# paolomandica/HALO

Measured on AMD Instinct MI355X. Metric: acquisition-scored images/sec (1024x2048, C=256, 19 cls), higher is better.
Workload: dtype f64

## Files before the change

halo_amd/csrc/halo_score.hip:

```cpp
#include "halo_common.hpp"
#include "halo_devmath.hpp"
#include "halo_select_plan.hpp"
#include "halo_softmax.hpp"
#include <stdlib.h>
#include <type_traits>

namespace halo {

constexpr int TPB = 256;
#ifndef HALO_FTPB
#define HALO_FTPB 128
#endif
#ifndef HALO_FEAT_WAVES
#define HALO_FEAT_WAVES 4
#endif
#ifndef HALO_FEAT_UNROLL
#define HALO_FEAT_UNROLL 8
#endif
constexpr int FTPB = HALO_FTPB;

__device__ __forceinline__ double nan_min(double a, double b) { return (a != a) ? a : ((b != b) ? b : (b < a ? b : a)); }
__device__ __forceinline__ double nan_max(double a, double b) { return (a != a) ? a : ((b != b) ? b : (b > a ? b : a)); }

template <int NT = TPB>
// ... 546 lines not shown
        unc[(size_t)b * hw + i] = a;
        mn = mx = (double)a;
    }
    if (!partials) return;
    __shared__ double seed[2];
    if (threadIdx.x == 0) { seed[0] = mn; seed[1] = mx; }
    __syncthreads();
    if (!live) { mn = seed[0]; mx = seed[1]; }
    block_minmax<TPB>(mn, mx, partials + ((size_t)b * gridDim.x + blockIdx.x) * 2);
}

__device__ __forceinline__ float lane_prev(float v)
{
    return __int_as_float(__builtin_amdgcn_update_dpp(0, __float_as_int(v), 0x138 , 0xf, 0xf, false));
}
__device__ __forceinline__ float lane_next(float v)
{
    return __int_as_float(__builtin_amdgcn_update_dpp(0, __float_as_int(v), 0x130 , 0xf, 0xf, false));
}

__device__ __forceinline__ float box3_over_count(float a, int H, int W, int y, int xx, int pk)
{
    if (pk <= 0) return a;
    const int rr = pk / 2;
    const int y0 = y - rr < 0 ? 0 : y - rr, y1 = y + rr >= H ? H - 1 : y + rr;
    const int x0 = xx - rr < 0 ? 0 : xx - rr, x1 = xx + rr >= W ? W - 1 : xx + rr;
    return a / (float)((y1 - y0 + 1) * (x1 - x0 + 1));
}

__device__ __forceinline__ void box3_row4(const float *__restrict__ ep, int H, int W, int y, int x, bool live, int pk, float (&o)[4])
{
    const int lane = threadIdx.x & 63;
    float r[3][6];
#pragma unroll
    for (int dy = 0; dy < 3; ++dy) {
        const int yy = y + dy - 1;
        const bool in = live && yy >= 0 && yy < H;
        const float *row = ep + (size_t)(in ? yy : 0) * W;
        float4 q = make_float4(0.0f, 0.0f, 0.0f, 0.0f);
        if (in) q = *reinterpret_cast<const float4 *>(row + x);
        float left = lane_prev(q.w), right = lane_next(q.x);
        if (lane == 0) left = (in && x > 0) ? row[x - 1] : 0.0f;
        if (lane == 63) right = (in && x + 4 < W) ? row[x + 4] : 0.0f;
        r[dy][0] = (in && x > 0) ? left : 0.0f;
        r[dy][1] = q.x; r[dy][2] = q.y; r[dy][3] = q.z; r[dy][4] = q.w;
        r[dy][5] = (in && x + 4 < W) ? right : 0.0f;
    }
#pragma unroll
    for (int j = 0; j < 4; ++j) {
        float a = 0.0f;
#pragma unroll
        for (int dy = 0; dy < 3; ++dy)
#pragma unroll
            for (int dx = 0; dx < 3; ++dx) a = a + r[dy][j + dx];
        o[j] = box3_over_count(a, H, W, y, x + j, pk);
    }
}

__global__ void __launch_bounds__(TPB) k_box3_unc(const float *__restrict__ ent, int H, int W, int pk,
                                                  float *__restrict__ unc, double *__restrict__ partials)
{
    const int b = blockIdx.y;
    const long long hw = (long long)H * W;
    const long long i0 = ((long long)blockIdx.x * TPB + threadIdx.x) * 4;
    const bool live = i0 < hw;
    double mn = 0.0, mx = 0.0;
    const int y = live ? (int)(i0 / W) : 0, x = live ? (int)(i0 % W) : 0;
    float o[4];
    box3_row4(ent + (size_t)b * hw, H, W, y, x, live, pk, o);
    if (live) {
        if (unc) *reinterpret_cast<float4 *>(unc + (size_t)b * hw + i0) = make_float4(o[0], o[1], o[2], o[3]);
        mn = mx = (double)o[0];
#pragma unroll
        for (int j = 1; j < 4; ++j) { mn = nan_min(mn, (double)o[j]); mx = nan_max(mx, (double)o[j]); }
    }
    if (!partials) return;
    __shared__ double seed[2];
    if (threadIdx.x == 0) { seed[0] = mn; seed[1] = mx; }
    __syncthreads();
    if (!live) { mn = seed[0]; mx = seed[1]; }
    block_minmax<TPB>(mn, mx, partials + ((size_t)b * gridDim.x + blockIdx.x) * 2);
}

constexpr int BM_RPT = 4, BM_TW = 256, BM_TH = BM_RPT * (TPB / 64);

__device__ __forceinline__ float nan_minf(float a, float b) { return (a != a) ? a : ((b != b) ? b : (b < a ? b : a)); }
__device__ __forceinline__ float nan_maxf(float a, float b) { return (a != a) ? a : ((b != b) ? b : (b > a ? b : a)); }

__global__ void __launch_bounds__(TPB) k_box3_minmax(const float *__restrict__ ent, int H, int W, int pk, double *__restrict__ partials,
                                                     unsigned *__restrict__ hist_zero)
{
    const int b = blockIdx.z, lane = threadIdx.x & 63, wv = threadIdx.x >> 6;
    if (hist_zero) {
        const unsigned nb = gridDim.x * gridDim.y;
        for (unsigned l = blockIdx.y * gridDim.x + blockIdx.x; l < NB1 / TPB; l += nb) hist_zero[(size_t)b * NB1 + l * TPB + threadIdx.x] = 0u;
    }
    const int x = blockIdx.x * BM_TW + lane * 4, y0 = blockIdx.y * BM_TH + wv * BM_RPT;
    const float *ep = ent + (size_t)b * H * W;
    const bool xin = x < W;
    auto load_row = [&](int yy, float (&r)[6]) {
        const bool in = xin && yy >= 0 && yy < H;
        const float *row = ep + (size_t)(in ? yy : 0) * W;
        float4 q = make_float4(0.0f, 0.0f, 0.0f, 0.0f);
        if (in) q = *reinterpret_cast<const float4 *>(row + x);
        float left = lane_prev(q.w), right = lane_next(q.x);
        if (lane == 0) left = (in && x > 0) ? row[x - 1] : 0.0f;
        if (lane == 63) right = (in && x + 4 < W) ? row[x + 4] : 0.0f;
        r[0] = (in && x > 0) ? left : 0.0f;
        r[1] = q.x; r[2] = q.y; r[3] = q.z; r[4] = q.w;
        r[5] = (in && x + 4 < W) ? right : 0.0f;
    };
    float r0[6], r1[6], r2[6];
    load_row(y0 - 1, r0);
    load_row(y0, r1);
    float mn = 0.0f, mx = 0.0f;
    bool have = false;
#pragma unroll
    for (int k = 0; k < BM_RPT; ++k) {
        const int y = y0 + k;
        load_row(y + 1, r2);
        if (xin && y < H) {
#pragma unroll
            for (int j = 0; j < 4; ++j) {
                float a = 0.0f;
#pragma unroll
                for (int dx = 0; dx < 3; ++dx) a = a + r0[j + dx];
#pragma unroll
                for (int dx = 0; dx < 3; ++dx) a = a + r1[j + dx];
#pragma unroll
                for (int dx = 0; dx < 3; ++dx) a = a + r2[j + dx];
                const float o = box3_over_count(a, H, W, y, x + j, pk);
                if (!have) { mn = mx = o; have = true; }
                else { mn = nan_minf(mn, o); mx = nan_maxf(mx, o); }
            }
        }
#pragma unroll
        for (int q = 0; q < 6; ++q) { r0[q] = r1[q]; r1[q] = r2[q]; }
    }
    __shared__ float seedf[2];
    __shared__ float smn[TPB / 64], smx[TPB / 64];
    if (threadIdx.x == 0) { seedf[0] = mn; seedf[1] = mx; }
    __syncthreads();
    if (!have) { mn = seedf[0]; mx = seedf[1]; }
#pragma unroll
    for (int off = 32; off > 0; off >>= 1) {
        mn = nan_minf(mn, __shfl_xor(mn, off));
        mx = nan_maxf(mx, __shfl_xor(mx, off));
    }
    if (lane == 0) { smn[wv] = mn; smx[wv] = mx; }
    __syncthreads();
    if (threadIdx.x == 0) {
#pragma unroll
        for (int i = 1; i < TPB / 64; ++i) { mn = nan_minf(mn, smn[i]); mx = nan_maxf(mx, smx[i]); }
        double *out2 = partials + (((size_t)b * gridDim.y + blockIdx.y) * gridDim.x + blockIdx.x) * 2;
        out2[0] = (double)mn;
        out2[1] = (double)mx;
    }
}

__global__ void __launch_bounds__(TPB) k_minmax_f32(const float *__restrict__ x, long long hw,
                                                    double *__restrict__ partials)
{
    const int b = blockIdx.y;
    const long long i = (long long)blockIdx.x * TPB + threadIdx.x;
    const bool live = i < hw;
    double mn = 0.0, mx = 0.0;
    if (live) mn = mx = (double)x[(size_t)b * hw + i];
    __shared__ double seed[2];
    if (threadIdx.x == 0) { seed[0] = mn; seed[1] = mx; }
    __syncthreads();
    if (!live) { mn = seed[0]; mx = seed[1]; }
    block_minmax<TPB>(mn, mx, partials + ((size_t)b * gridDim.x + blockIdx.x) * 2);
}

__global__ void __launch_bounds__(TPB) k_fill_f32(float *__restrict__ x, long long n, float v)
{
    const long long i = (long long)blockIdx.x * TPB + threadIdx.x;
    if (i < n) x[i] = v;
}

template <typename TI>
__global__ void __launch_bounds__(TPB) k_combine(const TI *__restrict__ imp_raw, const float *__restrict__ unc_raw,
                                                 const double *__restrict__ stats, const unsigned char *__restrict__ active,
                                                 long long hw, int normalize, TI *__restrict__ score,
                                                 TI *__restrict__ imp_out, float *__restrict__ unc_out)
{
    const int b = blockIdx.y;
    const long long i = (long long)blockIdx.x * TPB + threadIdx.x;
    if (i >= hw) return;
    const size_t o = (size_t)b * hw + i;
    TI im = imp_raw[o];
    float un = unc_raw[o];
    if (normalize) {
        const float umn = (float)stats[b * 4 + 2], umx = (float)stats[b * 4 + 3];
        un = (un - umn) / (float)((double)umx - (double)umn);
        const TI imn = (TI)stats[b * 4 + 0], imx = (TI)stats[b * 4 + 1];
        if constexpr (sizeof(TI) == 8) im = (im - imn) / (imx - imn);
        else im = (im - imn) / (float)((double)imx - (double)imn);
    }
    TI s = im * (TI)un;
    if (active && active[o]) {
        if constexpr (sizeof(TI) == 8) s = __longlong_as_double(0xfff0000000000000ll);
        else s = __uint_as_float(0xff800000u);
    }
    score[o] = s;
    if (imp_out) imp_out[o] = im;
    if (unc_out) unc_out[o] = un;
}


constexpr int CB_ROWS = 16;

template <typename TI>
__global__ void __launch_bounds__(TPB) k_combine_box3(const TI *__restrict__ imp_raw, const float *__restrict__ ent,
                                                      const double *__restrict__ stats, const unsigned char *__restrict__ active,
                                                      int H, int W, int pk, int normalize, TI *__restrict__ score,
                                                      TI *__restrict__ imp_out, float *__restrict__ unc_out, SelHdr *__restrict__ rng,
                                                      unsigned *__restrict__ hist, int rows)
{
    __shared__ unsigned hl[NB1];
    const int b = blockIdx.z;
    const long long hw = (long long)H * W;
    const int x = (blockIdx.x * TPB + threadIdx.x) * 4;
    const bool live = x < W;
    float umn = 0.0f, uden = 1.0f;
    TI imn = (TI)0, iden = (TI)1;
    bool fin = false;
    if (normalize) {
        umn = (float)stats[b * 4 + 2];
        const float umx = (float)stats[b * 4 + 3];
        uden = (float)((double)umx - (double)umn);
        imn = (TI)stats[b * 4 + 0];
        const TI imx = (TI)stats[b * 4 + 1];
        if constexpr (sizeof(TI) == 8) iden = imx - imn;
        else iden = (float)((double)imx - (double)imn);
        fin = uden > 0.0f && uden < __builtin_inff() && iden > (TI)0 && iden < (TI)__builtin_inf();
        if (rng && blockIdx.x == 0 && blockIdx.y == 0 && threadIdx.x == 0) {
            SelHdr h;
            memset(&h, 0, sizeof(h));
            h.kmin_inv = ~order_key(0.0);
            h.kmax = order_key(1.0);
            h.nvalid = 1u;
            h.flags = fin ? (hist ? (unsigned)SEL_F_HIST : 0u) : (unsigned)SEL_F_BAD;
            rng[b] = h;
        }
    }
    const bool count = hist != nullptr && fin;
    if (count) {
        for (int j = threadIdx.x; j < NB1; j += TPB) hl[j] = 0u;
        __syncthreads();
    }
    ValRange vr;
    vr.lo = 0.0; vr.scale = (double)NB1; vr.ok = true;
    const int ybeg = blockIdx.y * rows, yend = ybeg + rows < H ? ybeg + rows : H;
    const float *ep = ent + (size_t)b * hw;
    const int lane = threadIdx.x & 63;
    struct RowRaw { float4 q; float el, er; bool in; };
    auto row_issue = [&](int yy) {
        RowRaw t;
        t.in = live && yy >= 0 && yy < H;
        const float *row = ep + (size_t)(t.in ? yy : 0) * W;
        t.q = make_float4(0.0f, 0.0f, 0.0f, 0.0f);
        t.el = 0.0f; t.er = 0.0f;
        if (t.in) t.q = *reinterpret_cast<const float4 *>(row + x);
        if (lane == 0 && t.in && x > 0) t.el = row[x - 1];
        if (lane == 63 && t.in && x + 4 < W) t.er = row[x + 4];
        return t;
    };
    auto row_finish = [&](const RowRaw &t, float (&r)[6]) {
        float left = lane_prev(t.q.w), right = lane_next(t.q.x);
        if (lane == 0) left = t.el;
        if (lane == 63) right = t.er;
        r[0] = (t.in && x > 0) ? left : 0.0f;
        r[1] = t.q.x; r[2] = t.q.y; r[3] = t.q.z; r[4] = t.q.w;
        r[5] = (t.in && x + 4 < W) ? right : 0.0f;
    };
    typedef double cb_d2 __attribute__((ext_vector_type(2)));
    typedef float cb_f4 __attribute__((ext_vector_type(4)));
    struct PixRaw { cb_d2 d0, d1; cb_f4 f; unsigned am; };
    auto pix_issue = [&](int yy) {
        PixRaw t;
        t.d0 = (cb_d2){0.0, 0.0}; t.d1 = t.d0; t.f = (cb_f4){0.f, 0.f, 0.f, 0.f}; t.am = 0u;
        if (!live || yy >= yend) return t;
        const size_t o = (size_t)b * hw + (size_t)yy * W + x;
        if constexpr (sizeof(TI) == 8) {
            t.d0 = *reinterpret_cast<const cb_d2 *>(imp_raw + o);
            t.d1 = *reinterpret_cast<const cb_d2 *>(imp_raw + o + 2);
        } else {
            t.f = *reinterpret_cast<const cb_f4 *>(imp_raw + o);
        }
        if (active) t.am = *reinterpret_cast<const unsigned *>(active + o);
        return t;
    };
    float r0[6], r1[6], r2[6];
    {
        const RowRaw a0 = row_issue(ybeg - 1), a1 = row_issue(ybeg);
        row_finish(a0, r0);
        row_finish(a1, r1);
    }
    RowRaw nrow = row_issue(ybeg + 1);
    PixRaw npix = pix_issue(ybeg);
    for (int y = ybeg; y < yend; ++y) {
        row_finish(nrow, r2);
        const PixRaw cpix = npix;
        nrow = row_issue(y + 2);
        npix = pix_issue(y + 1);
        float un[4];
#pragma unroll
        for (int j = 0; j < 4; ++j) {
            float a = 0.0f;
#pragma unroll
            for (int dx = 0; dx < 3; ++dx) a = a + r0[j + dx];
#pragma unroll
            for (int dx = 0; dx < 3; ++dx) a = a + r1[j + dx];
#pragma unroll
            for (int dx = 0; dx < 3; ++dx) a = a + r2[j + dx];
// ... 840 lines not shown
    const Taps<float> ty = make_taps<float>(y, sh, h), tx = make_taps<float>(x, sw, w);
    const float *lb = logit + (size_t)b * bstride;
    for (int c = 0; c < O; ++c) {
        const float *pl = lb + (size_t)c * h * w;
        dst[((size_t)b * O + c) * hw + i] = bilerp<float>(pl[(size_t)ty.i0 * w + tx.i0], pl[(size_t)ty.i0 * w + tx.i1],
                                                          pl[(size_t)ty.i1 * w + tx.i0], pl[(size_t)ty.i1 * w + tx.i1], tx.l0, tx.l1, ty.l0, ty.l1);
    }
}

static inline bool aligned16(const void *p) { return ((uintptr_t)p & 15) == 0; }

struct FusedLogit { const float *logit; long long bstride; int O; int unc_type; float *ent; };

template <typename T, int VEC>
static void launch_feat(const T *feat, long long bstride, int C, long long hw, int B, int mode, double ks, double rks,
                        T *out, double *partials, int nblk, hipStream_t st, const FusedLogit *fl)
{
    dim3 grid(nblk, B), block(FTPB);
    constexpr int UNROLL = HALO_FEAT_UNROLL;
    unsigned xcd_g = 256;
    while (xcd_g > 1 && 8 * xcd_g > (unsigned)nblk) xcd_g >>= 1;
    if (8 * xcd_g > (unsigned)nblk) xcd_g = 0;
#define HALO_FEAT(M, FO_)                                                                                               \
    hipLaunchKernelGGL((k_feat_reduce<T, VEC, M, UNROLL, FO_>), grid, block, 0, st, feat, bstride, C, hw, ks, rks, out, \
                       partials, fl ? fl->logit : nullptr, fl ? fl->bstride : 0ll, fl ? fl->unc_type : 0, fl ? fl->ent : nullptr, \
                       xcd_g)
    const int fo = fl ? fl->O : 0;
    if (mode == 0) {
        if (fo == 19) HALO_FEAT(0, 19); else if (fo == 16) HALO_FEAT(0, 16); else HALO_FEAT(0, 0);
    } else {
        if (fo == 19) HALO_FEAT(1, 19); else if (fo == 16) HALO_FEAT(1, 16); else HALO_FEAT(1, 0);
    }
#undef HALO_FEAT
}

}

using namespace halo;

static_assert(RI_TW == LR_TW && RI_TH == LR_TH, "k_region_impurity3 writes one min/max partial per tile of the same shape");
static size_t partial_slots(int64_t H, int64_t W)
{
    const size_t a = (size_t)cdiv(H * W, FTPB), b = (size_t)(cdiv(W, LR_TW) * cdiv(H, LR_TH));
    return a > b ? a : b;
}

extern "C" size_t halo_score_workspace_bytes(int64_t B, int64_t H, int64_t W)
{
    if (B <= 0 || H <= 0 || W <= 0) return 0;
    const size_t n = (size_t)B * H * W;
    const size_t nblk = partial_slots(H, W);
    size_t s = 0;
    s += align_up(n * 4, 256);
    s += align_up(n * 4, 256);
    s += align_up(n * 8, 256);
    s += align_up(n * 2, 256);
    s += 2 * align_up((size_t)B * nblk * 2 * 8, 256);
    s += align_up((size_t)B * 4 * 8, 256);
    return s + 1024;
}

extern "C" size_t halo_score_args_workspace_bytes(const halo_score_args *a)
{
    if (!a || a->struct_bytes != sizeof(halo_score_args)) return 0;
    size_t s = halo_score_workspace_bytes(a->B, a->H, a->W);
    if (s == 0 || a->route == HALO_SCORE_FULL) return s;
    if (a->route != HALO_SCORE_LR && a->route != HALO_SCORE_LR_GRAM) return 0;
    if (a->O <= 0) return 0;
    if (!(a->O == 19 || a->O == 16)) s += (size_t)a->B * a->O * a->H * a->W * 4 + 512;
    if (a->route == HALO_SCORE_LR) return s;
    if (a->hf <= 0 || a->wf <= 0) return 0;
    return s + (size_t)a->B * 5 * a->hf * a->wf * 8 + 512;
}

static inline bool reads_feat(int pur_type) { return pur_type == HALO_PUR_HYPER || pur_type == HALO_PUR_RADIUS || pur_type == HALO_PUR_EUC_NORM; }
static inline bool is_ripu(int pur_type) { return pur_type == HALO_PUR_RIPU || pur_type == HALO_PUR_ORACLE_RIPU; }
static inline void record(void *event, hipStream_t st) { if (event) (void)hipEventRecord((hipEvent_t)event, st); }

struct ScorePlan {
    float *ent, *unc_raw;
    double *imp_raw;
    short *pred;
    double *part_imp, *part_unc, *stats;
    float *lr_logit_full;
    double *gram;
    bool lr, need_feat, hist, f64out, fuse;
    int pad, normalize, mode;
    double ks, rks;
    long long hw;
    int nblk1, nblk_imp, nblk_unc;
    FusedLogit fl;
};

template <typename T>
static void lr_window(int out_size, int in_size, int tile, int &max_span)
{
    const T sc = out_size > 1 ? (T)(in_size - 1) / (T)(out_size - 1) : (T)0;
    max_span = 1;
    for (int o0 = 0; o0 < out_size; o0 += tile) {
        const int ol = o0 + tile - 1 < out_size ? o0 + tile - 1 : out_size - 1;
        T f = sc * (T)o0; int lo = (int)f; lo = lo > in_size - 1 ? in_size - 1 : lo;
        f = sc * (T)ol; int hi = (int)f; hi = hi > in_size - 1 ? in_size - 1 : hi; hi = hi + (hi < in_size - 1 ? 1 : 0);
        if (hi - lo + 1 > max_span) max_span = hi - lo + 1;
    }
}

template <typename T>
static int launch_feat_lr(const halo_score_args &a, ScorePlan &p, T *out, hipStream_t st)
{
    const T *feat = (const T *)a.feat;
    const long long bstride = a.feat_bstride;
    const int C = (int)a.C, hf = (int)a.hf, wf = (int)a.wf, H = (int)a.H, W = (int)a.W, B = (int)a.B, mode = p.mode;
    const double ks = p.ks, rks = p.rks;
    double *partials = p.part_imp;
    int &nblk = p.nblk_imp;
    int max_rows, max_cols;
    lr_window<T>(H, hf, LR_TH, max_rows);
    lr_window<T>(W, wf, LR_TW, max_cols);
    ++max_rows; ++max_cols;
    const T sh = H > 1 ? (T)(hf - 1) / (T)(H - 1) : (T)0, sw = W > 1 ? (T)(wf - 1) / (T)(W - 1) : (T)0;
    dim3 grid((unsigned)cdiv(W, LR_TW), (unsigned)cdiv(H, LR_TH), (unsigned)B), block(TPB);
    nblk = (int)(grid.x * grid.y);
    auto with_mode = [mode](auto launch) {
        if (mode == 0) launch(std::integral_constant<int, 0>());
        else launch(std::integral_constant<int, 1>());
    };
    if constexpr (sizeof(T) == 8) {
        const int units_per_ch = max_rows * ((max_cols + 2) / 2 + 1);
        int CCd = DMA_UNITS / units_per_ch;
        CCd = CCd > C ? C : CCd;
        const bool dma_ok = wf >= 2 && wf % 2 == 0 && bstride % 2 == 0 && aligned16(feat) && CCd >= 4;
        if (dma_ok) {
            const size_t lds = 2 * (size_t)DMA_UNITS * 16;
            const int need_rows = max_rows, need_u = (max_cols + 2) / 2;
            if ((double)sh <= 1.0 / 3.0 && H >= 2 * LR_TH) {
                int max_rows8;
                lr_window<T>(H, hf, 2 * LR_TH, max_rows8);
                ++max_rows8;
                dim3 grid8((unsigned)cdiv(W, LR_TW), (unsigned)cdiv(H, 2 * LR_TH), (unsigned)B);
#define HALO_LR_FIXED8(R_, U_)                                                                                                             \
                if (max_rows8 <= R_ && need_u <= U_) {                                                                                     \
                    nblk = (int)(grid8.x * grid8.y);                                                                                       \
                    with_mode([&](auto M) { hipLaunchKernelGGL((k_feat_reduce_lr_dmaf<decltype(M)::value, R_, U_, 2 * LR_PPT>), grid8, block, lds, st, \
                                                               (const double *)feat, bstride, C, hf, wf, H, W, (double)sh, (double)sw, ks, rks, (double *)out, partials); }); \
                    return HALO_OK;                                                                                                       \
                }
                HALO_LR_FIXED8(8, 8)
                HALO_LR_FIXED8(11, 10)
#undef HALO_LR_FIXED8
            }
#define HALO_LR_FIXED(R_, U_)                                                                                                              \
            if (need_rows <= R_ && need_u <= U_) {                                                                                         \
                with_mode([&](auto M) { hipLaunchKernelGGL((k_feat_reduce_lr_dmaf<decltype(M)::value, R_, U_>), grid, block, lds, st,      \
                                                           (const double *)feat, bstride, C, hf, wf, H, W, (double)sh, (double)sw, ks, rks, (double *)out, partials); }); \
                return HALO_OK;                                                                                                            \
            }
            HALO_LR_FIXED(6, 8)
            HALO_LR_FIXED(7, 10)
            HALO_LR_FIXED(8, 12)
#undef HALO_LR_FIXED
            with_mode([&](auto M) { hipLaunchKernelGGL((k_feat_reduce_lr_dma<decltype(M)::value>), grid, block, lds, st,
                                                       (const double *)feat, bstride, C, hf, wf, H, W, (double)sh, (double)sw, CCd, ks, rks, (double *)out, partials); });
            return HALO_OK;
        }
    }
    const size_t plane_bytes = (size_t)max_rows * max_cols * sizeof(T);
    if (plane_bytes > 48 * 1024) return fail(HALO_E_UNSUPPORTED, "halo_score: source window too large for LDS (downsampling?)");
    int CC = (int)((48 * 1024) / plane_bytes);
    CC = CC > (TPB / 64) * LR_STAGE_G ? (TPB / 64) * LR_STAGE_G : CC;
    CC = CC > C ? C : CC;
    const size_t lds = (size_t)CC * plane_bytes;
    with_mode([&](auto M) { hipLaunchKernelGGL((k_feat_reduce_lr<T, decltype(M)::value>), grid, block, lds, st,
                                               feat, bstride, C, hf, wf, H, W, sh, sw, max_rows, max_cols, CC, ks, rks, out, partials); });
    return HALO_OK;
}

static int check_padding(int pad, int k, int64_t H, int64_t W, const char *who)
{
    if (pad < HALO_PAD_ZEROS || pad > HALO_PAD_CIRCULAR) return fail(HALO_E_ARG, "%s: bad padding mode %d", who, pad);
    const int64_t r = k / 2, m = H < W ? H : W;
    if (pad == HALO_PAD_REFLECT && r >= m)
        return fail(HALO_E_ARG, "%s: padding_mode='reflect' needs the padding (%lld) to be smaller than the map (%lld x %lld)", who, (long long)r, (long long)H, (long long)W);
    if (pad == HALO_PAD_CIRCULAR && r > m)
        return fail(HALO_E_ARG, "%s: padding_mode='circular' needs the padding (%lld) to be at most the map size (%lld x %lld)", who, (long long)r, (long long)H, (long long)W);
    return HALO_OK;
}

static int check_score_args(const halo_score_args &a)
{
    if (a.struct_bytes != sizeof(halo_score_args))
        return fail(HALO_E_ARG, "halo_score: descriptor of %zu bytes, this library reads %zu (another ABI?)", a.struct_bytes, sizeof(halo_score_args));
    if (a.route < HALO_SCORE_FULL || a.route > HALO_SCORE_LR_GRAM) return fail(HALO_E_ARG, "halo_score: unknown route %d", a.route);
    const bool need_feat = reads_feat(a.pur_type);
    if (a.route != HALO_SCORE_FULL) {
        if (a.hl <= 0 || a.wl <= 0) return fail(HALO_E_ARG, "halo_score: bad low-res logit size");
        if (need_feat && (a.hf <= 0 || a.wf <= 0)) return fail(HALO_E_ARG, "halo_score: bad low-res embedding size");
    }
    if (a.route == HALO_SCORE_LR_GRAM && need_feat) {
        if (a.hf * a.wf > 0x7fffffffll) return fail(HALO_E_UNSUPPORTED, "halo_score: low-res planes of more than 2^31 elements (Gram route)");
        if (a.workspace_bytes < halo_score_args_workspace_bytes(&a)) return fail(HALO_E_WORKSPACE, "halo_score: workspace too small for the Gram route");
    }
    if (a.flags & ~(HALO_FLAG_NORMALIZE | (3 << 8))) return fail(HALO_E_ARG, "halo_score: unknown flag bits 0x%x", a.flags);
    if (!a.logit || !a.score || a.B <= 0 || a.O <= 0 || a.H <= 0 || a.W <= 0) return fail(HALO_E_ARG, "halo_score: null/empty argument");
    if (a.unc_type < 0 || a.unc_type > HALO_UNC_ZEROS) return fail(HALO_E_ARG, "halo_score: bad unc_type %d", a.unc_type);
    if (a.pur_type < 0 || a.pur_type > HALO_PUR_EUC_NORM) return fail(HALO_E_UNSUPPORTED, "Error: purity type '%d' not implemented", a.pur_type);
    if (a.ksize < 1 || !(a.ksize & 1) || a.pksize < 1 || !(a.pksize & 1)) return fail(HALO_E_ARG, "halo_score: window sizes must be odd");
    const int rc = check_padding((a.flags >> 8) & 3, a.ksize > a.pksize ? a.ksize : a.pksize, a.H, a.W, "halo_score");
    if (rc != HALO_OK) return rc;
    if (need_feat && (!a.feat || a.C <= 0)) return fail(HALO_E_ARG, "halo_score: decoder_out required for this purity type");
    if (need_feat && a.feat_dtype != HALO_F32 && a.feat_dtype != HALO_F64) return fail(HALO_E_ARG, "halo_score: bad feat dtype");
    const bool need_gt = a.unc_type == HALO_UNC_ORACLE_ACC || a.pur_type == HALO_PUR_ORACLE_RIPU;
    if (need_gt && !a.gt) return fail(HALO_E_ARG, "halo_score: ground_truth required");
    if (a.pur_type == HALO_PUR_HYPER && (a.K < 1 || a.K > 32767)) return fail(HALO_E_UNSUPPORTED, "halo_score: K out of range");
    if (a.O > 32767) return fail(HALO_E_UNSUPPORTED, "halo_score: too many classes");
    const size_t base = halo_score_workspace_bytes(a.B, a.H, a.W);
    if (a.workspace_bytes < base || !a.workspace) return fail(HALO_E_WORKSPACE, "halo_score: workspace too small");
    if (a.route != HALO_SCORE_FULL && !(a.O == 19 || a.O == 16) && a.workspace_bytes < base + (size_t)a.B * a.O * a.H * a.W * 4 + 256)
        return fail(HALO_E_WORKSPACE, "halo_score: workspace too small for %d classes from low-res logits", (int)a.O);
    return HALO_OK;
}

static int make_score_plan(const halo_score_args &a, ScorePlan &p)
{
    const size_t B = (size_t)a.B;
    p.lr = a.route != HALO_SCORE_FULL;
    p.need_feat = reads_feat(a.pur_type);
    p.pad = (a.flags >> 8) & 3;
    p.normalize = a.flags & HALO_FLAG_NORMALIZE;
    p.hw = (long long)a.H * a.W;
    p.nblk1 = (int)cdiv(p.hw, TPB);
    p.nblk_imp = p.nblk_unc = p.nblk1;

    Arena ar(a.workspace, a.workspace_bytes);
    p.ent = ar.take<float>(B * p.hw);
    p.unc_raw = ar.take<float>(B * p.hw);
    p.imp_raw = ar.take<double>(B * p.hw);
    p.pred = ar.take<short>(B * p.hw);
    p.part_imp = ar.take<double>(B * partial_slots(a.H, a.W) * 2);
    p.part_unc = ar.take<double>(B * partial_slots(a.H, a.W) * 2);
    p.stats = ar.take<double>(B * 4);
    p.lr_logit_full = (p.lr && !(a.O == 19 || a.O == 16)) ? ar.take<float>(B * a.O * p.hw) : nullptr;
    const bool gram_mode = a.route == HALO_SCORE_LR_GRAM && p.need_feat;
    if (gram_mode && a.feat_dtype != HALO_F64) return fail(HALO_E_UNSUPPORTED, "halo_score: float64 embeddings only on the Gram route");
    p.gram = gram_mode ? ar.take<double>(B * GRAM_MAPS * a.hf * a.wf) : nullptr;
    if (!ar.ok()) return fail(HALO_E_WORKSPACE, "halo_score: workspace too small");

    p.f64out = (a.pur_type == HALO_PUR_RADIUS || a.pur_type == HALO_PUR_EUC_NORM) && a.feat_dtype == HALO_F64;
    p.hist = is_ripu(a.pur_type) || a.pur_type == HALO_PUR_HYPER;
    p.mode = a.pur_type == HALO_PUR_EUC_NORM ? 1 : 0;
    p.ks = sqrt(fabs(-a.c) + 1e-15);
    p.rks = 1.0 / p.ks;

    const bool ent_only = (a.unc_type == HALO_UNC_ENTROPY || a.unc_type == HALO_UNC_PIXEL_ENTROPY) && !is_ripu(a.pur_type);
    const int fvec = !p.need_feat ? 0 : (a.feat_dtype == HALO_F64
        ? (((p.hw % 2 == 0) && (a.feat_bstride % 2 == 0) && aligned16(a.feat) && aligned16(p.imp_raw)) ? 2 : 1)
        : (((p.hw % 4 == 0) && (a.feat_bstride % 4 == 0) && aligned16(a.feat) && aligned16(p.imp_raw)) ? 4 : 1));
    p.fuse = !p.lr && p.need_feat && ent_only && (a.O == 19 || a.O == 16) && fvec > 1 && (a.logit_bstride % fvec == 0) &&
             (((uintptr_t)a.logit) % (4 * fvec) == 0);
    p.fl = FusedLogit{a.logit, (long long)a.logit_bstride, (int)a.O, a.unc_type, p.ent};
    return HALO_OK;
}

static void launch_logit_pass(const halo_score_args &a, const ScorePlan &p, hipStream_t st)
{
    if (p.fuse) return;
    const int B = (int)a.B, O = (int)a.O, H = (int)a.H, W = (int)a.W;
    const long long hw = p.hw, bstride = a.logit_bstride;
    const long long *gt = (const long long *)a.gt;
    short *pred = is_ripu(a.pur_type) ? p.pred : nullptr;
    const dim3 block(TPB), grid1((unsigned)p.nblk1, (unsigned)B);
    if (a.unc_type == HALO_UNC_ZEROS && !is_ripu(a.pur_type)) {
        hipLaunchKernelGGL(k_fill_f32, dim3((unsigned)cdiv(B * hw, TPB)), block, 0, st, p.ent, (long long)(B * hw), 0.0f);
    } else if (p.lr) {
        const int hl = (int)a.hl, wl = (int)a.wl;
        const float shl = H > 1 ? (float)(hl - 1) / (float)(H - 1) : 0.0f, swl = W > 1 ? (float)(wl - 1) / (float)(W - 1) : 0.0f;
        if (O == 19)
            hipLaunchKernelGGL((k_logit_maps_lr<19>), grid1, block, 0, st, a.logit, bstride, hl, wl, H, W, shl, swl, gt, a.unc_type, a.pur_type, p.ent, pred);
        else if (O == 16)
            hipLaunchKernelGGL((k_logit_maps_lr<16>), grid1, block, 0, st, a.logit, bstride, hl, wl, H, W, shl, swl, gt, a.unc_type, a.pur_type, p.ent, pred);
        else {
            hipLaunchKernelGGL(k_logit_interp_lr, grid1, block, 0, st, a.logit, bstride, O, hl, wl, H, W, shl, swl, p.lr_logit_full);
            hipLaunchKernelGGL(k_logit_maps_generic, grid1, block, 0, st, (const float *)p.lr_logit_full, (long long)(O * hw), gt, O, hw, a.unc_type, a.pur_type, 0, p.ent, pred);
        }
    } else {
        const bool vec4 = (hw % 4 == 0) && (bstride % 4 == 0) && aligned16(a.logit) && aligned16(p.ent);
        const dim3 grid4((unsigned)cdiv(hw, TPB * 4), (unsigned)B);
        if (O == 19 && vec4)
            hipLaunchKernelGGL((k_logit_maps<19, 4>), grid4, block, 0, st, a.logit, bstride, gt, hw, a.unc_type, a.pur_type, p.ent, pred);
        else if (O == 16 && vec4)
            hipLaunchKernelGGL((k_logit_maps<16, 4>), grid4, block, 0, st, a.logit, bstride, gt, hw, a.unc_type, a.pur_type, p.ent, pred);
        else
            hipLaunchKernelGGL(k_logit_maps_generic, grid1, block, 0, st, a.logit, bstride, gt, O, hw, a.unc_type, a.pur_type, 0, p.ent, pred);
    }
}

static void launch_gram(const halo_score_args &a, const ScorePlan &p, hipStream_t st)
{
    const double *feat = (const double *)a.feat;
    const long long bstride = a.feat_bstride;
    const int B = (int)a.B, C = (int)a.C, H = (int)a.H, W = (int)a.W, hf = (int)a.hf, wf = (int)a.wf;
    const dim3 block(TPB);
    const bool wide = wf >= 2 && wf % 2 == 0 && bstride % 2 == 0 && aligned16(feat) && aligned16(p.gram);
    if (wide) {
        const long long nwx = cdiv(wf, 128);
        int rows = 2;
        for (int cand = 8; cand > 2; cand >>= 1)
            if (B * nwx * cdiv(hf, cand) >= 1024) { rows = cand; break; }
        const long long nwaves = nwx * cdiv(hf, rows);
        const dim3 gg((unsigned)(cdiv(cdiv(nwaves, TPB / 64), 8) * 8), (unsigned)B);
#define HALO_GRAM2(U_, R_) hipLaunchKernelGGL((k_gram_lr2<U_, R_>), gg, block, 0, st, feat, bstride, C, hf, wf, p.gram)
        if (rows == 8) HALO_GRAM2(1, 8);
        else if (rows == 4) HALO_GRAM2(2, 4);
        else HALO_GRAM2(2, 2);
#undef HALO_GRAM2
    } else {
        const long long nwaves = cdiv(wf, GRAM_COLS) * cdiv(hf, 2);
        hipLaunchKernelGGL(k_gram_lr, dim3((unsigned)(cdiv(cdiv(nwaves, TPB / 64), 8) * 8), (unsigned)B), block, 0, st, feat, bstride, C, hf, wf, p.gram);
    }
    record(a.ev_feat_mid, st);
    const double shd = H > 1 ? (double)(hf - 1) / (double)(H - 1) : 0.0, swd = W > 1 ? (double)(wf - 1) / (double)(W - 1) : 0.0;
    const dim3 grid1((unsigned)p.nblk1, (unsigned)B);
    if (p.mode == 0) hipLaunchKernelGGL(k_radius_gram<0>, grid1, block, 0, st, p.gram, feat, bstride, C, hf, wf, H, W, shd, swd, p.ks, p.rks, p.imp_raw, p.part_imp);
    else hipLaunchKernelGGL(k_radius_gram<1>, grid1, block, 0, st, p.gram, feat, bstride, C, hf, wf, H, W, shd, swd, p.ks, p.rks, p.imp_raw, p.part_imp);
}

static int launch_feature_pass(const halo_score_args &a, ScorePlan &p, hipStream_t st)
{
    const int B = (int)a.B, C = (int)a.C;
    const long long hw = p.hw, bstride = a.feat_bstride;
    if (p.gram) {
        launch_gram(a, p, st);
        p.nblk_imp = p.nblk1;
    } else if (p.lr) {
        return a.feat_dtype == HALO_F64 ? launch_feat_lr<double>(a, p, p.imp_raw, st)
                                        : launch_feat_lr<float>(a, p, (float *)p.imp_raw, st);
    } else if (a.feat_dtype == HALO_F64) {
        const bool v2 = (hw % 2 == 0) && (bstride % 2 == 0) && aligned16(a.feat) && aligned16(p.imp_raw);
        p.nblk_imp = (int)cdiv(hw, v2 ? FTPB * 2 : FTPB);
        if (v2) launch_feat<double, 2>((const double *)a.feat, bstride, C, hw, B, p.mode, p.ks, p.rks, p.imp_raw, p.part_imp, p.nblk_imp, st, p.fuse ? &p.fl : nullptr);
        else launch_feat<double, 1>((const double *)a.feat, bstride, C, hw, B, p.mode, p.ks, p.rks, p.imp_raw, p.part_imp, p.nblk_imp, st, nullptr);
    } else {
        const bool v4 = (hw % 4 == 0) && (bstride % 4 == 0) && aligned16(a.feat) && aligned16(p.imp_raw);
        p.nblk_imp = (int)cdiv(hw, v4 ? FTPB * 4 : FTPB);
        if (v4) launch_feat<float, 4>((const float *)a.feat, bstride, C, hw, B, p.mode, p.ks, p.rks, (float *)p.imp_raw, p.part_imp, p.nblk_imp, st, p.fuse ? &p.fl : nullptr);
        else launch_feat<float, 1>((const float *)a.feat, bstride, C, hw, B, p.mode, p.ks, p.rks, (float *)p.imp_raw, p.part_imp, p.nblk_imp, st, nullptr);
    }
    return HALO_OK;
}

static int launch_tail(const halo_score_args &a, ScorePlan &p, hipStream_t st)
{
    const int64_t B = a.B, H = a.H, W = a.W;
    const long long hw = p.hw;
    const int normalize = p.normalize, box_pk = p.hist ? a.pksize : 0;
    const dim3 block(TPB), grid1((unsigned)p.nblk1, (unsigned)B);
    if (a.pur_type == HALO_PUR_HYPER) {
        hipLaunchKernelGGL(k_minmax_finalize, dim3((unsigned)B), block, 0, st, p.part_imp, p.nblk_imp, p.stats, 0);
        if (a.feat_dtype == HALO_F64) hipLaunchKernelGGL((k_quantize<double, short>), grid1, block, 0, st, (const double *)p.imp_raw, p.stats, hw, (int)a.K, p.pred);
        else hipLaunchKernelGGL((k_quantize<float, short>), grid1, block, 0, st, (const float *)p.imp_raw, p.stats, hw, (int)a.K, p.pred);
    }
    if (p.hist) {
        const float logK = (float)log((double)(a.pur_type == HALO_PUR_HYPER ? a.K : a.O));
        const int np = launch_region_impurity<short>((const short *)p.pred, B, H, W, a.pksize, logK, (float *)p.imp_raw, (float *)nullptr, st,
                                                     normalize ? p.part_imp : nullptr, p.pad);
        p.nblk_imp = np ? np : p.nblk1;
        if (normalize && !np) hipLaunchKernelGGL(k_minmax_f32, grid1, block, 0, st, (const float *)p.imp_raw, hw, p.part_imp);
    } else if (a.pur_type == HALO_PUR_NONE) {
        hipLaunchKernelGGL(k_fill_f32, dim3((unsigned)cdiv(B * hw, TPB)), block, 0, st, (float *)p.imp_raw, (long long)(B * hw), 0.0f);
        if (normalize) hipLaunchKernelGGL(k_minmax_f32, grid1, block, 0, st, (const float *)p.imp_raw, hw, p.part_imp);
        p.nblk_imp = p.nblk1;
    }

    const int do_box = (a.unc_type == HALO_UNC_ENTROPY || a.unc_type == HALO_UNC_ORACLE_ACC) ? 1 : 0;
    const bool box3 = do_box && p.pad == HALO_PAD_ZEROS && a.ksize == 3 && W % 4 == 0 && aligned16(p.ent) && aligned16(p.unc_raw);
    const bool fuse_tail = box3 && B <= 65535 && H <= 65535 && aligned16(p.imp_raw) && aligned16(a.score) && (!a.impurity || aligned16(a.impurity)) &&
                           (!a.uncertainty || aligned16(a.uncertainty)) && (!a.active || ((uintptr_t)a.active & 3) == 0);
    SelHdr *rng_free = (a.score_range && normalize && fuse_tail) ? (SelHdr *)a.score_range : nullptr;
    unsigned *rng_hist = rng_free ? (unsigned *)((char *)a.score_range + range_hist_offset(B)) : nullptr;
    if (fuse_tail) {
        if (normalize) {
            const dim3 gridm((unsigned)cdiv(W, BM_TW), (unsigned)cdiv(H, BM_TH), (unsigned)B);
            p.nblk_unc = (int)(gridm.x * gridm.y);
            hipLaunchKernelGGL(k_box3_minmax, gridm, block, 0, st, (const float *)p.ent, (int)H, (int)W, box_pk, p.part_unc, rng_hist);
        }
    } else if (box3) {
        p.nblk_unc = (int)cdiv(hw, TPB * 4);
        hipLaunchKernelGGL(k_box3_unc, dim3((unsigned)p.nblk_unc, (unsigned)B), block, 0, st, (const float *)p.ent, (int)H, (int)W, box_pk, p.unc_raw,
                           normalize ? p.part_unc : nullptr);
    } else {
        hipLaunchKernelGGL(k_box_unc, grid1, block, 0, st, p.ent, (int)H, (int)W, a.ksize, do_box, box_pk, p.unc_raw, normalize ? p.part_unc : nullptr, p.pad);
    }

    if (normalize)
        hipLaunchKernelGGL(k_minmax_finalize2, dim3((unsigned)B, 2u), dim3(FIN_TPB), 0, st, (const double *)p.part_imp, p.nblk_imp,
                           (const double *)p.part_unc, p.nblk_unc, p.stats);
    if (fuse_tail) {
        int crows = CB_ROWS;
        while (crows > 1 && cdiv(W, TPB * 4) * cdiv(H, crows) * B < 1024) crows >>= 1;
        dim3 gridc((unsigned)cdiv(W, TPB * 4), (unsigned)cdiv(H, crows), (unsigned)B);
#define HALO_CB(T) hipLaunchKernelGGL((k_combine_box3<T>), gridc, block, 0, st, (const T *)p.imp_raw, (const float *)p.ent, p.stats, a.active, (int)H, (int)W, box_pk, normalize, (T *)a.score, (T *)a.impurity, a.uncertainty, rng_free, rng_hist, crows)
        if (p.f64out) HALO_CB(double);
        else HALO_CB(float);
#undef HALO_CB
    } else if (p.f64out) hipLaunchKernelGGL((k_combine<double>), grid1, block, 0, st, (const double *)p.imp_raw, p.unc_raw, p.stats, a.active, hw, normalize, (double *)a.score, (double *)a.impurity, a.uncertainty);
    else hipLaunchKernelGGL((k_combine<float>), grid1, block, 0, st, (const float *)p.imp_raw, p.unc_raw, p.stats, a.active, hw, normalize, (float *)a.score, (float *)a.impurity, a.uncertainty);
    if (a.score_range && !rng_free) {
        const int rc = score_range_exact(a.score, p.f64out ? HALO_F64 : HALO_F32, B, hw, a.score_range, st);
        if (rc != HALO_OK) return rc;
    }
    record(a.ev_tail_stop, st);
    return check_launch("halo_score");
}

static int score_impl(const halo_score_args &a, hipStream_t st)
{
    ScorePlan p;
    int rc = check_score_args(a);
    if (rc == HALO_OK) rc = make_score_plan(a, p);
    if (rc != HALO_OK) return rc;

    record(a.ev_logit_start, st);
    launch_logit_pass(a, p, st);
    record(a.ev_logit_stop, st);
    if (p.need_feat) {
        record(a.ev_feat_start, st);
        rc = launch_feature_pass(a, p, st);
        if (rc != HALO_OK) return rc;
        record(a.ev_feat_stop, st);
    }
    if (a.tail_stream && (hipStream_t)a.tail_stream != st) {
        if (!p.need_feat || !a.ev_feat_stop) return fail(HALO_E_ARG, "halo_score: a purity type that reads decoder_out and ev_feat_stop are required with a tail stream");
        if (hipStreamWaitEvent((hipStream_t)a.tail_stream, (hipEvent_t)a.ev_feat_stop, 0) != hipSuccess)
            return fail(HALO_E_LAUNCH, "halo_score: hipStreamWaitEvent: %s", hipGetErrorString(hipGetLastError()));
        st = (hipStream_t)a.tail_stream;
    }
    return launch_tail(a, p, st);
}

extern "C" int halo_score(const halo_score_args *a, void *stream)
{
    if (!a) return fail(HALO_E_ARG, "halo_score: null descriptor");
    return score_impl(*a, (hipStream_t)stream);
}

extern "C" int halo_region_uncertainty(const float *x, int64_t bstride, int is_prob, const int64_t *gt, int64_t B, int64_t O,
                                       int64_t H, int64_t W, int unc_type, int ksize, int do_box, float *out,
                                       void *workspace, size_t workspace_bytes, void *stream)
{
    hipStream_t st = (hipStream_t)stream;
    const int pad = (do_box >> 8) & 3;
    do_box &= 1;
    if (!x || !out || B <= 0 || O <= 0 || H <= 0 || W <= 0) return fail(HALO_E_ARG, "halo_region_uncertainty: null/empty argument");
    if (unc_type < 0 || unc_type > HALO_UNC_ZEROS) return fail(HALO_E_ARG, "halo_region_uncertainty: bad unc_type");
    if (unc_type == HALO_UNC_ORACLE_ACC && !gt) return fail(HALO_E_ARG, "halo_region_uncertainty: ground_truth required");
    if (ksize < 1 || !(ksize & 1)) return fail(HALO_E_ARG, "halo_region_uncertainty: window size must be odd");
    if (do_box) { const int rc = check_padding(pad, ksize, H, W, "halo_region_uncertainty"); if (rc != HALO_OK) return rc; }
    const long long hw = (long long)H * W;
    if (!workspace || workspace_bytes < (size_t)B * hw * 4 + 256) return fail(HALO_E_WORKSPACE, "halo_region_uncertainty: workspace too small");
    float *ent = (float *)(((uintptr_t)workspace + 255) & ~(uintptr_t)255);
    dim3 block(TPB), grid1((unsigned)cdiv(hw, TPB), (unsigned)B);
    float *dst = do_box ? ent : out;
    if (unc_type == HALO_UNC_ZEROS)
        hipLaunchKernelGGL(k_fill_f32, dim3((unsigned)cdiv(B * hw, TPB)), block, 0, st, dst, (long long)(B * hw), 0.0f);
    else
        hipLaunchKernelGGL(k_logit_maps_generic, grid1, block, 0, st, x, (long long)bstride, (const long long *)gt, (int)O, hw,
                           unc_type, HALO_PUR_NONE, is_prob, dst, (short *)nullptr);
    if (do_box)
        hipLaunchKernelGGL(k_box_unc, grid1, block, 0, st, (const float *)ent, (int)H, (int)W, ksize, 1, 0, out, (double *)nullptr, pad);
    return check_launch("halo_region_uncertainty");
}

extern "C" int halo_region_impurity(const int64_t *pred, int64_t B, int64_t H, int64_t W, int ksize, int64_t K, float *impurity,
                                    float *count, int pad_mode, void *stream)
{
    if (!pred || !impurity || B <= 0 || H <= 0 || W <= 0 || K < 1) return fail(HALO_E_ARG, "halo_region_impurity: null/empty argument");
    if (ksize < 1 || !(ksize & 1)) return fail(HALO_E_ARG, "halo_region_impurity: window size must be odd");
    { const int rc = check_padding(pad_mode, ksize, H, W, "halo_region_impurity"); if (rc != HALO_OK) return rc; }
    launch_region_impurity<long long>((const long long *)pred, B, H, W, ksize, (float)log((double)K), impurity, count, (hipStream_t)stream,
                                      nullptr, pad_mode);
    return check_launch("halo_region_impurity");
}

extern "C" int halo_quantize_radius(const void *feat, int feat_dtype, int64_t feat_bstride, int64_t B, int64_t C, int64_t H,
// ... 28 lines not shown
```

Measured before the change: 1354.

## Fold minmax finalize into box3 minmax and combine kernels with persistent tiling

```diff
diff --git a/halo_amd/csrc/halo_score.hip b/halo_amd/csrc/halo_score.hip
--- a/halo_amd/csrc/halo_score.hip
+++ b/halo_amd/csrc/halo_score.hip
@@ -652,63 +652,109 @@
     block_minmax<TPB>(mn, mx, partials + ((size_t)b * gridDim.x + blockIdx.x) * 2);
 }
 
-constexpr int BM_RPT = 4, BM_TW = 256, BM_TH = BM_RPT * (TPB / 64);
+constexpr int BM_CH = 2, BM_TW = 256, BM_ROWS = 16, BM_WAVES = TPB / 64;
+constexpr int FIN_WAVES = FIN_TPB / 64;
+constexpr int BM_MAX_WG = 256;
 
 __device__ __forceinline__ float nan_minf(float a, float b) { return (a != a) ? a : ((b != b) ? b : (b < a ? b : a)); }
 __device__ __forceinline__ float nan_maxf(float a, float b) { return (a != a) ? a : ((b != b) ? b : (b > a ? b : a)); }
 
 __global__ void __launch_bounds__(TPB) k_box3_minmax(const float *__restrict__ ent, int H, int W, int pk, double *__restrict__ partials,
-                                                     unsigned *__restrict__ hist_zero)
-{
-    const int b = blockIdx.z, lane = threadIdx.x & 63, wv = threadIdx.x >> 6;
+                                                     unsigned *__restrict__ hist_zero, const double *__restrict__ part_imp, int nblk_imp,
+                                                     double *__restrict__ sec_imp, int nsec)
+{
+    const int b = blockIdx.y, g = blockIdx.x, G = gridDim.x, lane = threadIdx.x & 63, wv = threadIdx.x >> 6;
     if (hist_zero) {
-        const unsigned nb = gridDim.x * gridDim.y;
-        for (unsigned l = blockIdx.y * gridDim.x + blockIdx.x; l < NB1 / TPB; l += nb) hist_zero[(size_t)b * NB1 + l * TPB + threadIdx.x] = 0u;
-    }
-    const int x = blockIdx.x * BM_TW + lane * 4, y0 = blockIdx.y * BM_TH + wv * BM_RPT;
+        for (int l = g; l < NB1 / TPB; l += G) hist_zero[(size_t)b * NB1 + l * TPB + threadIdx.x] = 0u;
+    }
+    const int slot = g * BM_WAVES + wv, nslots = G * BM_WAVES;
+    if (part_imp) {
+        const int spread = G / FIN_WAVES;
+        const double2 *p = reinterpret_cast<const double2 *>(part_imp + (size_t)b * nblk_imp * 2);
+        for (int w = 0; w < nsec; ++w) {
+            const int owner = spread >= 1 ? w * spread * BM_WAVES + (BM_WAVES - 1) : w % nslots;
+            if (owner != slot) continue;
+            const double2 p0 = p[0];
+            double mn = p0.x, mx = p0.y;
+            for (int i = w * 64 + lane; i < nblk_imp; i += FIN_TPB) { const double2 q = p[i]; mn = nan_min(mn, q.x); mx = nan_max(mx, q.y); }
+#pragma unroll
+            for (int off = 32; off > 0; off >>= 1) {
+                mn = nan_min(mn, __shfl_xor(mn, off));
+                mx = nan_max(mx, __shfl_xor(mx, off));
+            }
+            if (lane == 0) {
+                double *o = sec_imp + ((size_t)b * nsec + w) * 2;
+                o[0] = mn;
+                o[1] = mx;
+            }
+        }
+    }
     const float *ep = ent + (size_t)b * H * W;
-    const bool xin = x < W;
-    auto load_row = [&](int yy, float (&r)[6]) {
-        const bool in = xin && yy >= 0 && yy < H;
-        const float *row = ep + (size_t)(in ? yy : 0) * W;
-        float4 q = make_float4(0.0f, 0.0f, 0.0f, 0.0f);
-        if (in) q = *reinterpret_cast<const float4 *>(row + x);
-        float left = lane_prev(q.w), right = lane_next(q.x);
-        if (lane == 0) left = (in && x > 0) ? row[x - 1] : 0.0f;
-        if (lane == 63) right = (in && x + 4 < W) ? row[x + 4] : 0.0f;
-        r[0] = (in && x > 0) ? left : 0.0f;
-        r[1] = q.x; r[2] = q.y; r[3] = q.z; r[4] = q.w;
-        r[5] = (in && x + 4 < W) ? right : 0.0f;
+    struct RowRaw { float4 q; float el, er; bool in; };
+    auto row_issue = [&](int yy, int x, bool xin) {
+        RowRaw t;
+        t.in = xin && yy >= 0 && yy < H;
+        const float *row = ep + (size_t)(t.in ? yy : 0) * W;
+        t.q = make_float4(0.0f, 0.0f, 0.0f, 0.0f);
+        t.el = 0.0f; t.er = 0.0f;
+        if (t.in) t.q = *reinterpret_cast<const float4 *>(row + x);
+        if (lane == 0 && t.in && x > 0) t.el = row[x - 1];
+        if (lane == 63 && t.in && x + 4 < W) t.er = row[x + 4];
+        return t;
     };
-    float r0[6], r1[6], r2[6];
-    load_row(y0 - 1, r0);
-    load_row(y0, r1);
+    auto row_finish = [&](const RowRaw &t, int x, float (&r)[6]) {
+        float left = lane_prev(t.q.w), right = lane_next(t.q.x);
+        if (lane == 0) left = t.el;
+        if (lane == 63) right = t.er;
+        r[0] = (t.in && x > 0) ? left : 0.0f;
+        r[1] = t.q.x; r[2] = t.q.y; r[3] = t.q.z; r[4] = t.q.w;
+        r[5] = (t.in && x + 4 < W) ? right : 0.0f;
+    };
+    const int ntx = (W + BM_TW - 1) / BM_TW, nt = ntx * ((H + BM_ROWS - 1) / BM_ROWS);
     float mn = 0.0f, mx = 0.0f;
     bool have = false;
-#pragma unroll
-    for (int k = 0; k < BM_RPT; ++k) {
-        const int y = y0 + k;
-        load_row(y + 1, r2);
-        if (xin && y < H) {
-#pragma unroll
-            for (int j = 0; j < 4; ++j) {
-                float a = 0.0f;
-#pragma unroll
-                for (int dx = 0; dx < 3; ++dx) a = a + r0[j + dx];
-#pragma unroll
-                for (int dx = 0; dx < 3; ++dx) a = a + r1[j + dx];
-#pragma unroll
-                for (int dx = 0; dx < 3; ++dx) a = a + r2[j + dx];
-                const float o = box3_over_count(a, H, W, y, x + j, pk);
-                if (!have) { mn = mx = o; have = true; }
-                else { mn = nan_minf(mn, o); mx = nan_maxf(mx, o); }
-            }
-        }
-#pragma unroll
-        for (int q = 0; q < 6; ++q) { r0[q] = r1[q]; r1[q] = r2[q]; }
+    for (int t = slot; t < nt; t += nslots) {
+        const int ty = t / ntx, tx = t - ty * ntx;
+        const int x = tx * BM_TW + lane * 4, y0 = ty * BM_ROWS;
+        const int yend = y0 + BM_ROWS < H ? y0 + BM_ROWS : H;
+        const bool xin = x < W;
+        float r0[6], r1[6], r2[6];
+        RowRaw ring[BM_CH];
+        {
+            const RowRaw a0 = row_issue(y0 - 1, x, xin), a1 = row_issue(y0, x, xin);
+#pragma unroll
+            for (int k = 0; k < BM_CH; ++k) ring[k] = row_issue(y0 + 1 + k, x, xin);
+            row_finish(a0, x, r0);
+            row_finish(a1, x, r1);
+        }
+        for (int yc = y0; yc < yend; yc += BM_CH) {
+#pragma unroll
+            for (int k = 0; k < BM_CH; ++k) {
+                const int y = yc + k;
+                row_finish(ring[k], x, r2);
+                if (y + 1 + BM_CH <= yend) ring[k] = row_issue(y + 1 + BM_CH, x, xin);
+                if (xin && y < yend) {
+#pragma unroll
+                    for (int j = 0; j < 4; ++j) {
+                        float a = 0.0f;
+#pragma unroll
+                        for (int dx = 0; dx < 3; ++dx) a = a + r0[j + dx];
+#pragma unroll
+                        for (int dx = 0; dx < 3; ++dx) a = a + r1[j + dx];
+#pragma unroll
+                        for (int dx = 0; dx < 3; ++dx) a = a + r2[j + dx];
+                        const float o = box3_over_count(a, H, W, y, x + j, pk);
+                        if (!have) { mn = mx = o; have = true; }
+                        else { mn = nan_minf(mn, o); mx = nan_maxf(mx, o); }
+                    }
+                }
+#pragma unroll
+                for (int q = 0; q < 6; ++q) { r0[q] = r1[q]; r1[q] = r2[q]; }
+            }
+        }
     }
     __shared__ float seedf[2];
-    __shared__ float smn[TPB / 64], smx[TPB / 64];
+    __shared__ float smn[BM_WAVES], smx[BM_WAVES];
     if (threadIdx.x == 0) { seedf[0] = mn; seedf[1] = mx; }
     __syncthreads();
     if (!have) { mn = seedf[0]; mx = seedf[1]; }
@@ -721,8 +767,8 @@
     __syncthreads();
     if (threadIdx.x == 0) {
 #pragma unroll
-        for (int i = 1; i < TPB / 64; ++i) { mn = nan_minf(mn, smn[i]); mx = nan_maxf(mx, smx[i]); }
-        double *out2 = partials + (((size_t)b * gridDim.y + blockIdx.y) * gridDim.x + blockIdx.x) * 2;
+        for (int i = 1; i < BM_WAVES; ++i) { mn = nan_minf(mn, smn[i]); mx = nan_maxf(mx, smx[i]); }
+        double *out2 = partials + ((size_t)b * G + g) * 2;
         out2[0] = (double)mn;
         out2[1] = (double)mx;
     }
@@ -783,7 +829,9 @@
 
 template <typename TI>
 __global__ void __launch_bounds__(TPB) k_combine_box3(const TI *__restrict__ imp_raw, const float *__restrict__ ent,
-                                                      const double *__restrict__ stats, const unsigned char *__restrict__ active,
+                                                      double *__restrict__ stats, const double *__restrict__ sec_imp,
+                                                      int nsec, const double *__restrict__ part_unc, int nunc,
+                                                      const unsigned char *__restrict__ active,
                                                       int H, int W, int pk, int normalize, TI *__restrict__ score,
                                                       TI *__restrict__ imp_out, float *__restrict__ unc_out, SelHdr *__restrict__ rng,
                                                       unsigned *__restrict__ hist, int rows)
@@ -797,11 +845,29 @@
     TI imn = (TI)0, iden = (TI)1;
     bool fin = false;
     if (normalize) {
-        umn = (float)stats[b * 4 + 2];
-        const float umx = (float)stats[b * 4 + 3];
+        const int lane = threadIdx.x & 63;
+        const double2 *si = reinterpret_cast<const double2 *>(sec_imp) + (size_t)b * nsec;
+        const double2 *pu = reinterpret_cast<const double2 *>(part_unc) + (size_t)b * nunc;
+        const double2 i0 = si[0], u0 = pu[0];
+        double imnd = i0.x, imxd = i0.y;
+        for (int i = 1; i < nsec; ++i) { const double2 q = si[i]; imnd = nan_min(imnd, q.x); imxd = nan_max(imxd, q.y); }
+        float umx = (float)u0.y;
+        umn = (float)u0.x;
+        for (int i = lane; i < nunc; i += 64) { const double2 q = pu[i]; umn = nan_minf(umn, (float)q.x); umx = nan_maxf(umx, (float)q.y); }
+#pragma unroll
+        for (int off = 32; off > 0; off >>= 1) {
+            umn = nan_minf(umn, __shfl_xor(umn, off));
+            umx = nan_maxf(umx, __shfl_xor(umx, off));
+        }
+        umn = __shfl(umn, 0);
+        umx = __shfl(umx, 0);
+        if (blockIdx.x == 0 && blockIdx.y == 0 && threadIdx.x == 0) {
+            stats[b * 4 + 0] = imnd; stats[b * 4 + 1] = imxd;
+            stats[b * 4 + 2] = (double)umn; stats[b * 4 + 3] = (double)umx;
+        }
         uden = (float)((double)umx - (double)umn);
-        imn = (TI)stats[b * 4 + 0];
-        const TI imx = (TI)stats[b * 4 + 1];
+        imn = (TI)imnd;
+        const TI imx = (TI)imxd;
         if constexpr (sizeof(TI) == 8) iden = imx - imn;
         else iden = (float)((double)imx - (double)imn);
         fin = uden > 0.0f && uden < __builtin_inff() && iden > (TI)0 && iden < (TI)__builtin_inf();
@@ -1808,6 +1874,7 @@
     double *imp_raw;
     short *pred;
     double *part_imp, *part_unc, *stats;
+    double *sec_imp;
     float *lr_logit_full;
     double *gram;
     bool lr, need_feat, hist, f64out, fuse;
@@ -1965,6 +2032,7 @@
     p.part_imp = ar.take<double>(B * partial_slots(a.H, a.W) * 2);
     p.part_unc = ar.take<double>(B * partial_slots(a.H, a.W) * 2);
     p.stats = ar.take<double>(B * 4);
+    p.sec_imp = reinterpret_cast<double *>(p.unc_raw);
     p.lr_logit_full = (p.lr && !(a.O == 19 || a.O == 16)) ? ar.take<float>(B * a.O * p.hw) : nullptr;
     const bool gram_mode = a.route == HALO_SCORE_LR_GRAM && p.need_feat;
     if (gram_mode && a.feat_dtype != HALO_F64) return fail(HALO_E_UNSUPPORTED, "halo_score: float64 embeddings only on the Gram route");
@@ -2099,15 +2167,21 @@
 
     const int do_box = (a.unc_type == HALO_UNC_ENTROPY || a.unc_type == HALO_UNC_ORACLE_ACC) ? 1 : 0;
     const bool box3 = do_box && p.pad == HALO_PAD_ZEROS && a.ksize == 3 && W % 4 == 0 && aligned16(p.ent) && aligned16(p.unc_raw);
+    const int nsec = (int)(cdiv(p.nblk_imp, 64) < FIN_WAVES ? cdiv(p.nblk_imp, 64) : FIN_WAVES);
     const bool fuse_tail = box3 && B <= 65535 && H <= 65535 && aligned16(p.imp_raw) && aligned16(a.score) && (!a.impurity || aligned16(a.impurity)) &&
-                           (!a.uncertainty || aligned16(a.uncertainty)) && (!a.active || ((uintptr_t)a.active & 3) == 0);
+                           (!a.uncertainty || aligned16(a.uncertainty)) && (!a.active || ((uintptr_t)a.active & 3) == 0) &&
+                           (long long)nsec * 16 <= hw * 4;
     SelHdr *rng_free = (a.score_range && normalize && fuse_tail) ? (SelHdr *)a.score_range : nullptr;
     unsigned *rng_hist = rng_free ? (unsigned *)((char *)a.score_range + range_hist_offset(B)) : nullptr;
     if (fuse_tail) {
         if (normalize) {
-            const dim3 gridm((unsigned)cdiv(W, BM_TW), (unsigned)cdiv(H, BM_TH), (unsigned)B);
-            p.nblk_unc = (int)(gridm.x * gridm.y);
-            hipLaunchKernelGGL(k_box3_minmax, gridm, block, 0, st, (const float *)p.ent, (int)H, (int)W, box_pk, p.part_unc, rng_hist);
+            const int64_t ntiles = cdiv(W, BM_TW) * cdiv(H, BM_ROWS);
+            int64_t wgs = 2048 / B;
+            wgs = wgs < 1 ? 1 : (wgs > BM_MAX_WG ? BM_MAX_WG : wgs);
+            if (wgs > cdiv(ntiles, BM_WAVES)) wgs = cdiv(ntiles, BM_WAVES);
+            p.nblk_unc = (int)wgs;
+            hipLaunchKernelGGL(k_box3_minmax, dim3((unsigned)wgs, (unsigned)B), block, 0, st, (const float *)p.ent, (int)H, (int)W, box_pk, p.part_unc,
+                               rng_hist, (const double *)p.part_imp, p.nblk_imp, p.sec_imp, nsec);
         }
     } else if (box3) {
         p.nblk_unc = (int)cdiv(hw, TPB * 4);
@@ -2117,14 +2191,14 @@
         hipLaunchKernelGGL(k_box_unc, grid1, block, 0, st, p.ent, (int)H, (int)W, a.ksize, do_box, box_pk, p.unc_raw, normalize ? p.part_unc : nullptr, p.pad);
     }
 
-    if (normalize)
+    if (normalize && !fuse_tail)
         hipLaunchKernelGGL(k_minmax_finalize2, dim3((unsigned)B, 2u), dim3(FIN_TPB), 0, st, (const double *)p.part_imp, p.nblk_imp,
                            (const double *)p.part_unc, p.nblk_unc, p.stats);
     if (fuse_tail) {
         int crows = CB_ROWS;
         while (crows > 1 && cdiv(W, TPB * 4) * cdiv(H, crows) * B < 1024) crows >>= 1;
         dim3 gridc((unsigned)cdiv(W, TPB * 4), (unsigned)cdiv(H, crows), (unsigned)B);
-#define HALO_CB(T) hipLaunchKernelGGL((k_combine_box3<T>), gridc, block, 0, st, (const T *)p.imp_raw, (const float *)p.ent, p.stats, a.active, (int)H, (int)W, box_pk, normalize, (T *)a.score, (T *)a.impurity, a.uncertainty, rng_free, rng_hist, crows)
+#define HALO_CB(T) hipLaunchKernelGGL((k_combine_box3<T>), gridc, block, 0, st, (const T *)p.imp_raw, (const float *)p.ent, p.stats, (const double *)p.sec_imp, nsec, (const double *)p.part_unc, p.nblk_unc, a.active, (int)H, (int)W, box_pk, normalize, (T *)a.score, (T *)a.impurity, a.uncertainty, rng_free, rng_hist, crows)
         if (p.f64out) HALO_CB(double);
         else HALO_CB(float);
 #undef HALO_CB
```

Result: no change. 1358, median of 6 (+0.3%).
